# leijue222/Intra-and-Inter-Human-Relation-Network-for-MPEE

Hardware: AMD Instinct MI355X
Metric: images/sec (256x192 crops) I2R-Net HRNet-W48 inference (higher is better)
Workload: dtype f32; 1 GPU; vanilla I2R-Net HRNet-W48-S 256x192, 6 encoder layers, fp32, random weights (BASELINE configs[1]: w48_pure_en6); images_per_gpu=8, persons_per_image=4, crops_per_gpu_step=32, parallelism=single GPU, programs_per_forward=3

## Files before the change

### include/i2r_hip.h

```cpp
#ifndef I2R_HIP_H
#define I2R_HIP_H

#include <stdint.h>

#ifdef __cplusplus
extern "C" {
#endif

#define I2R_ABI_VERSION 17

#define I2R_API __attribute__((visibility("default")))

#define I2R_OK 0
#define I2R_E_ARG (-1)
#define I2R_E_LAUNCH (-2)
#define I2R_E_NODEV (-3)

#define I2R_MAX_TAPS 9

typedef struct i2r_conv_desc {
    const float* in;
    const float* in2;
    const float* w;
    const float* bias;
// ... 39 lines not shown

I2R_API int i2r_pe_res_stem(const float* mask_nchw, const float* w_pre, const float* w7, const float* bias, float* out_nhwc,
                    int32_t n_img, int32_t in_h, int32_t in_w, int32_t cout, int32_t out_cs, int32_t n_src, int32_t n_valid, void* stream);

typedef struct i2r_pe_cat_vec_args {
    const float* in; const float* w; const float* bias; float* out;
    int32_t n_img, in_h, in_w, th, tw, rate, vec, out_cs, c0, c_end, n_src, n_valid;
} i2r_pe_cat_vec_args;
I2R_API int i2r_pe_cat_vec(const i2r_pe_cat_vec_args* a, void* stream);

I2R_API int i2r_maxpool3x3s2(const float* in, float* out, int32_t n_img, int32_t in_h, int32_t in_w, int32_t c,
                     int32_t in_cs, int32_t out_cs, void* stream);

I2R_API int i2r_head(const float* in, const float* w, const float* bias, float* out_nchw, int32_t n_img, int32_t h,
             int32_t w_, int32_t cin, int32_t in_cs, int32_t cout, void* stream);

I2R_API int i2r_conv_kernel_name(const i2r_conv_desc* const* descs, int32_t n, char* buf, int32_t buflen);

I2R_API int i2r_conv_grid(const i2r_conv_desc* const* descs, int32_t n, int32_t with_map, int32_t* grid, int32_t* seq);

I2R_API int i2r_conv_wino_form(const i2r_conv_desc* const* descs, int32_t n, int32_t* form);
I2R_API int i2r_conv_wino_forms(int32_t on);

I2R_API int i2r_flip_merge(const float* y, const float* y_flipped, const int32_t* joint_map, float* out, int32_t n, int32_t joints,
                   int32_t h, int32_t w, void* stream);

I2R_API int i2r_decode(const float* heatmaps, const float* center, const float* scale, float* preds, float* maxvals, int32_t n,
               int32_t joints, int32_t h, int32_t w, int32_t blur_kernel, int32_t transform_back, void* stream);

#define I2R_MAX_TOKEN_TABLES 2
typedef struct i2r_token_table { int32_t* tokens; const int32_t* crop_group; const int32_t* crop_slot; int32_t n_grp, K, fh, fw, down, reserved; } i2r_token_table;
typedef struct i2r_joint_tokens_args {
    const float* heatmaps; float* points; float* maxvals; i2r_token_table table[I2R_MAX_TOKEN_TABLES ];
    int32_t n_crops, joints, hh, hw, in_stride, n_tables;
} i2r_joint_tokens_args;
I2R_API int i2r_joint_tokens(const i2r_joint_tokens_args* a, void* stream);

typedef struct i2r_pose_nms_args {
    const float* preds; const float* maxvals; const float* scale; const float* area; const float* box_score;
    const int32_t* img_off; const float* sigmas;
    float* score; int32_t* rank; int32_t* n_keep;
    double in_vis_thre, oks_thre, oks_vis_thre;
    int32_t n_crops, n_img, joints, max_persons, soft, max_dets, use_oks_vis, reserved;
} i2r_pose_nms_args;
I2R_API int i2r_pose_nms(const i2r_pose_nms_args* a, void* stream);

// ... 289 lines not shown
```

### intra-and-inter-human-relation-network-for-mpee_amd/cabi.py

```python
import ctypes as C
import os

import torch

_HERE = os.path.dirname(os.path.abspath(__file__))
LIB_PATH = os.path.join(_HERE, "libi2r_hip.so")

MAX_TAPS = 9
ABI_VERSION = 17
OP_CONV, OP_STEM, OP_MAXPOOL, OP_HEAD, OP_ENC_KV, OP_ENC_LAYER, OP_FORK, OP_JOIN, OP_CONV_GROUP = 1, 2, 3, 4, 5, 6, 7, 8, 9
MAX_GROUP = 4
OP_LAYERNORM, OP_WINATTN, OP_DWCONV, OP_UPSAMPLE = 10, 11, 12, 13
OP_CONV_CHAIN = 14
OP_PE_RES_STEM = 15
OP_HRT_ATTN = 16
OP_HRT_MLP = 17
OP_XSYNC = 18
OP_FUSE_UP = 19
OP_CONV1X1_PAIR = 20
OP_CONV1X1_LP = 21
OP_MH_ATTN = 22
OP_PE_CAT_VEC = 23
OP_ROWS_GATHER, OP_VIEW_SCRAMBLE = 24, 25
OP_RECORD, OP_WAIT = 26, 27
# ... 213 lines not shown
    _fields_ = [("output", _fp), ("target", _fp), ("target_weight", _fp), ("joints_hm", _fp), ("joints_vis", _fp), ("joints_weight", _fp),
                ("ws", _fp), ("loss", _fp), ("acc", _fp), ("avg_acc", _fp), ("cnt", _fp), ("pred", _fp), ("sse", _fp), ("hits", _fp),
                ("valid", _fp), ("meter", _fp), ("sigma", C.c_double),
                ("n_crops", _i32), ("joints", _i32), ("h", _i32), ("w", _i32), ("use_target_weight", _i32), ("reserved", _i32)]


class ValCombineArgs(C.Structure):
    _fields_ = [("parts", _fp), ("sse", _fp), ("hits", _fp), ("valid", _fp), ("loss", _fp), ("acc", _fp), ("avg_acc", _fp), ("cnt", _fp),
                ("n_crops", _fp), ("meter", _fp), ("n_part", _i32), ("joints", _i32), ("h", _i32), ("w", _i32)]


class ImageRef(C.Structure):
    _fields_ = [("img", C.c_void_p), ("ih", _i32), ("iw", _i32), ("row_bytes", _i32), ("reserved", _i32)]


class CropRef(C.Structure):
    _fields_ = [("inv_m", C.c_double * 6), ("box", _i32 * 4), ("image", _i32), ("reserved", _i32 * 3)]


class Op(C.Structure):
    _fields_ = [("kind", _i32), ("lane", _i32), ("args", C.c_void_p)]


EXPORTS = ("i2r_conv", "i2r_conv_grouped", "i2r_conv_kernel_name", "i2r_conv_grid", "i2r_conv_wino_form", "i2r_conv_wino_forms", "i2r_stem_conv", "i2r_pe_res_stem", "i2r_maxpool3x3s2", "i2r_head", "i2r_layernorm", "i2r_window_attn", "i2r_hrt_attn_block", "i2r_hrt_mlp_block", "i2r_dwconv3x3",
           "i2r_upsample_bilinear_add", "i2r_upsample_bilinear_add_multi", "i2r_fuse_up_add", "i2r_conv1x1_pair", "i2r_conv1x1_lp", "i2r_flip_merge", "i2r_decode", "i2r_joint_tokens", "i2r_pose_nms", "i2r_group_nearest", "i2r_oks_match", "i2r_oks_accumulate", "i2r_joint_targets", "i2r_val_metrics", "i2r_val_combine", "i2r_crop_affine", "i2r_box_mask", "i2r_crop_affine_cv2", "i2r_box_mask_cv2", "i2r_person_inputs_cv2", "i2r_encoder_kv", "i2r_encoder_layer", "i2r_mh_attention", "i2r_attn_weights", "i2r_attn_query_maps", "i2r_attn_person_maps", "i2r_attn_flip_merge", "i2r_token_mirror", "i2r_pe_cat_vec", "i2r_rows_gather", "i2r_rows_gather_multi", "i2r_view_scramble",
           "i2r_run_program", "i2r_run_program_timed", "i2r_abi_version", "i2r_last_error", "i2r_device_check")

_LIB = None


class I2RError(RuntimeError):
    pass


def load_library(path=LIB_PATH):
    if not os.path.exists(path):
        raise I2RError(
            "HIP extension %s is missing -- build it with `python -c 'import __graft_entry__ as g; g.build()'`. "
            "There is no CPU fallback for the product path." % path)
    L = C.CDLL(path)
    L.i2r_conv.argtypes = [C.POINTER(ConvDesc), C.c_void_p]
    L.i2r_conv_grouped.argtypes = [C.POINTER(C.POINTER(ConvDesc)), _i32, _fp, _i32, C.c_void_p]
    L.i2r_conv_kernel_name.argtypes = [C.POINTER(C.POINTER(ConvDesc)), _i32, C.c_char_p, _i32]
    L.i2r_conv_grid.argtypes = [C.POINTER(C.POINTER(ConvDesc)), _i32, _i32, C.POINTER(_i32), C.POINTER(_i32)]
    L.i2r_conv_wino_form.argtypes = [C.POINTER(C.POINTER(ConvDesc)), _i32, C.POINTER(_i32)]
    L.i2r_conv_wino_forms.argtypes = [_i32]
    L.i2r_stem_conv.argtypes = [_fp, _fp, _fp, _fp, _i32, _i32, _i32, _i32, _i32, _i32, _i32, _i32, _i32, C.c_void_p]
    L.i2r_pe_res_stem.argtypes = [_fp, _fp, _fp, _fp, _fp, _i32, _i32, _i32, _i32, _i32, _i32, _i32, C.c_void_p]
    L.i2r_flip_merge.argtypes = [_fp, _fp, _fp, _fp, _i32, _i32, _i32, _i32, C.c_void_p]
    L.i2r_decode.argtypes = [_fp, _fp, _fp, _fp, _fp, _i32, _i32, _i32, _i32, _i32, _i32, C.c_void_p]
    L.i2r_joint_tokens.argtypes = [C.POINTER(JointTokensArgs), C.c_void_p]
    L.i2r_pose_nms.argtypes = [C.POINTER(PoseNmsArgs), C.c_void_p]
    L.i2r_group_nearest.argtypes = [_fp, _fp, _fp, _i32, _i32, _i32, _i32, _fp, C.c_void_p]
    L.i2r_oks_match.argtypes = [C.POINTER(OksMatchArgs), C.c_void_p]
    L.i2r_oks_accumulate.argtypes = [C.POINTER(OksAccumulateArgs), C.c_void_p]
    L.i2r_joint_targets.argtypes = [C.POINTER(JointTargetsArgs), C.c_void_p]
    L.i2r_val_metrics.argtypes = [C.POINTER(ValMetricsArgs), C.c_void_p]
    L.i2r_val_combine.argtypes = [C.POINTER(ValCombineArgs), C.c_void_p]
    L.i2r_crop_affine.argtypes = [_fp, _i32, _i32, _i32, _i32, _fp, _fp, _fp, _fp, _i32, _i32, _i32, C.c_void_p]
    L.i2r_box_mask.argtypes = [_fp, _i32, _i32, _fp, _i32, _i32, _i32, C.c_void_p]
    L.i2r_crop_affine_cv2.argtypes = [_fp, _i32, _i32, _i32, _i32, _fp, _fp, _fp, _fp, _i32, _i32, _i32, C.c_void_p]
    L.i2r_box_mask_cv2.argtypes = [_fp, _i32, _i32, _fp, _i32, _i32, _i32, C.c_void_p]
    L.i2r_person_inputs_cv2.argtypes = [_fp, _i32, _fp, _i32, _i32, C.POINTER(C.c_float), C.POINTER(C.c_float), _fp, _fp, _i32, _i32, C.c_void_p]
    L.i2r_fuse_up_add.argtypes = [_fp, _fp, _i32, _fp, _i32, _fp, _i32, _i32, _i32, _i32, _i32, _i32, C.c_void_p]
    L.i2r_conv1x1_pair.argtypes = [C.POINTER(Conv1x1PairArgs), C.c_void_p]
    L.i2r_conv1x1_lp.argtypes = [C.POINTER(Conv1x1LpArgs), C.c_void_p]
    L.i2r_maxpool3x3s2.argtypes = [_fp, _fp, _i32, _i32, _i32, _i32, _i32, _i32, C.c_void_p]
    L.i2r_head.argtypes = [_fp, _fp, _fp, _fp, _i32, _i32, _i32, _i32, _i32, _i32, C.c_void_p]
    L.i2r_layernorm.argtypes = [_fp, _fp, _fp, _fp, _i32, _i32, _i32, C.c_float, _i32, C.c_void_p]
# ... 49 lines not shown
```

### intra-and-inter-human-relation-network-for-mpee_amd/csrc/i2r_conv.h

```cpp
#pragma once
#include "i2r_common.h"

#ifdef I2R_TUNING
#define I2R_DBG(p) ((p).dbg)
#else
#define I2R_DBG(p) 0
#endif

namespace {

struct ConvK {
    const float* in;
    const float* in2;
    const float* w;
    const float* bias;
    const float* res1;
    const float* res2;
    const float* res_post;
    float* out;
    int n_img, in_h, in_w, in_cs, cin;
    int conv_h, conv_w, out_h, out_w, out_cs, cout, cout_pad;
    int stride, iy0, ix0, ntaps;
    int tap_kh, tap_kw;
    int out_step, out_off_y, out_off_x, rep, relu;
// ... 223 lines not shown
    for (int mt = 0; mt < MT; ++mt) {
        const int m = (wm * MT + mt) * 16 + g * 4 + pj;
        const int ty = div_m(m, p.tile_w, p.m_tw), tx = m - ty * p.tile_w;
        const int oy = oy0 + ty, ox = ox0 + tx;
        const bool pvalid = m < tile_px && oy < p.conv_h && ox < p.conv_w;
        const int by = oy * p.out_step + p.out_off_y, bx = ox * p.out_step + p.out_off_x;
#pragma unroll
        for (int nt = 0; nt < NT; ++nt) {
            const f32x4 v = to_pixel_major(acc[mt][nt]) + bias[nt];
            const int n = n_base + nt * 16 + pq * 4;
            if (!pvalid || noff[nt] == kOOB) continue;
            for (int ry = 0; ry < p.rep; ++ry)
                for (int rx = 0; rx < p.rep; ++rx) {
                    const unsigned o = (unsigned)(((img * p.out_h + by + ry) * p.out_w + bx + rx) * p.out_cs) * esz + noff[nt];
                    f32x4 t = v;
                    if (p.res1) t += buf_ld_act4<DT>(rs_r1, o, h16);
                    if (p.res2) t += buf_ld_act4<DT>(rs_r2, o, h16);
                    buf_st_act4<DT>(rs_out, o, finish(t, n, n + 4 <= p.cout, o), h16);
                }
        }
    }
}



typedef void (*conv_fn)(const ConvGroupK);

}

void* i2r_pick_conv_f32(int nt, int mt, int cap, int pf);
void* i2r_pick_conv_bf16(int nt, int mt, int cap, int pf);
void* i2r_pick_conv_f16(int nt, int mt, int cap, int pf);
void* i2r_pick_conv_wino(int nt, int mt, int fin, int epi);
size_t i2r_conv_wino_lds(int nt, int mt, int plane);
```

### intra-and-inter-human-relation-network-for-mpee_amd/csrc/i2r_conv.hip

```cpp
#include "i2r_conv.h"

namespace {

template <int MT, int NT, int CAP, int PF>
__device__ __forceinline__ void conv_body(const ConvK& p, int bid, f32x4* lds) {
    const int tid = threadIdx.x;
    unsigned long long ts0 = 0, ts1 = 0, ts2 = 0;
    const bool stamp = (I2R_DBG(p) & 8) != 0;
    const int bid_stamp = bid;
    if (stamp) ts0 = __builtin_amdgcn_s_memtime();
    const int lane = tid & 63, wave = tid >> 6;
    const int WN = p.wn;
    const int wm = wave >> p.wn_log, wn = wave & (WN - 1);
    const int li = lane & 15, g = lane >> 4;

    int q = div_m(bid, p.n_cblk, p.m_cblk);
    const int cb = bid - q * p.n_cblk;
    bid = q;
    q = div_m(bid, p.tiles_x, p.m_tx);
    const int tile_x = bid - q * p.tiles_x;
    bid = q;
    const int img = div_m(bid, p.tiles_y, p.m_ty);
    const int tile_y = bid - img * p.tiles_y;
    const int oy0 = tile_y * p.tile_h, ox0 = tile_x * p.tile_w;
// ... 162 lines not shown
    }

    if (stamp) {
        ts2 = __builtin_amdgcn_s_memtime();
        ConvK q = p;
        q.res2 = nullptr;
        conv_epilogue<MT, NT, 0>(q, acc, img, oy0, ox0, wm, n_base, li, g, tile_px);
        asm volatile("s_waitcnt vmcnt(0)" ::: "memory");
        const unsigned long long ts3 = __builtin_amdgcn_s_memtime();
        if (tid == 0) {
            unsigned long long* o = reinterpret_cast<unsigned long long*>(const_cast<float*>(p.res2)) + (size_t)bid_stamp * 4;
            o[0] = ts0; o[1] = ts1; o[2] = ts2; o[3] = ts3;
            if (I2R_DBG(p) & 32) {
                const unsigned hw = __builtin_amdgcn_s_getreg((4 << 0) | (0 << 6) | (31 << 11));
                const unsigned xcc = __builtin_amdgcn_s_getreg((20 << 0) | (0 << 6) | (3 << 11));
                o[1] = ((unsigned long long)xcc << 32) | hw;
            }
        }
        return;
    }
    conv_epilogue<MT, NT, 0>(p, acc, img, oy0, ox0, wm, n_base, li, g, tile_px);
}

template <int MT, int NT, int CAP, int PF>
__global__ __launch_bounds__(256) void conv_igemm_f32(const ConvGroupK grp) {
    extern __shared__ __attribute__((aligned(16))) f32x4 lds[];
    int bid = blockIdx.x, gi = 0, start = 0;
    if (grp.blk_map) {
        const int v = __builtin_amdgcn_readfirstlane(grp.blk_map[bid]);
        gi = v >> 24;
        bid = v & 0xFFFFFF;
    } else {
#pragma unroll
        for (int i = 0; i < kMaxGroups - 1; ++i)
            if (i + 1 < grp.n && bid >= grp.blk_end[i]) { gi = i + 1; start = grp.blk_end[i]; }
    }
    conv_body<MT, NT, CAP, PF>(grp.g[gi], bid - start, lds);
}

template <int NT, int CAP, int PF>
conv_fn pick_mt(int mt) {
    switch (mt) {
        case 1: return conv_igemm_f32<1, NT, CAP, PF>;
        case 2: return conv_igemm_f32<2, NT, CAP, PF>;
        case 3: return conv_igemm_f32<3, NT, CAP, PF>;
        case 4: return conv_igemm_f32<4, NT, CAP, PF>;
    }
    return nullptr;
}

template <int CAP, int PF>
conv_fn pick_nt(int nt, int mt) {
    switch (nt) {
        case 3: return pick_mt<3, CAP, PF>(mt);
        case 4: return pick_mt<4, CAP, PF>(mt);
        case 5: return pick_mt<5, CAP, PF>(mt);
    }
    return nullptr;
}

}

void* i2r_pick_conv_f32(int nt, int mt, int cap, int pf) {
    conv_fn fn = nullptr;
    if (pf == 0) fn = pick_nt<4, 0>(nt, mt);
    if (pf == 1 && cap == 4) fn = pick_nt<4, 1>(nt, mt);
    if (pf == 1 && cap == 12) fn = pick_nt<12, 1>(nt, mt);
    if (pf == 2 && cap == 4) fn = pick_nt<4, 2>(nt, mt);
    return reinterpret_cast<void*>(fn);
}

#include "i2r_conv_plan.h"
```

### intra-and-inter-human-relation-network-for-mpee_amd/csrc/i2r_conv_plan.h

```cpp
#pragma once
#include <stdlib.h>

#include <algorithm>
#include <atomic>

#include "i2r_conv.h"

namespace {

inline int cdiv(int a, int b) { return (a + b - 1) / b; }
inline unsigned magic(int d) { return d == 1 ? 0u : (unsigned)(((1ull << 32) + d - 1) / d); }
inline unsigned recip31(int d) { return (unsigned)(((1ull << 31) + d - 1) / d); }

struct ConvTune { int dbg, plane_pad, pf, cap; };
#ifdef I2R_TUNING
inline const ConvTune& conv_tune() {
    auto env = [](const char* name, int dflt) { const char* v = getenv(name); return v ? atoi(v) : dflt; };
    static const ConvTune t = {env("I2R_CONV_DBG", 0), env("I2R_CONV_PLANE_PAD", 0), env("I2R_CONV_PF", 1), env("I2R_CONV_CAP", 12)};
    return t;
}
#else
constexpr ConvTune conv_tune() { return {0, 0, 1, 12}; }
#endif

struct ConvShape {
    int nt, wn, mt;
    int tile_h, tile_w, tiles_y, tiles_x, n_cblk;
    int tap_kh, tap_kw, ph, pw, plane;
    int npp, cin_g, g_ch;
    int cap, pf, ck;
    unsigned in_bytes, w_bytes, out_bytes;
    size_t lds;
    long long nblk;
};

struct ConvPlan {
    ConvGroupK grp;
    int algo, dtype;
    int nt, mt, cap, pf;
    bool fused_in; int form;
    size_t lds; long long total;
    int seq[kMaxGroups];
    conv_fn fn;
};

void copy_desc(const i2r_conv_desc* d, ConvK& k) {
    k = ConvK{};
    k.in = d->in; k.in2 = d->in2; k.w = d->w; k.bias = d->bias; k.res1 = d->res1; k.res2 = d->res2; k.res_post = d->res_post; k.out = d->out;
    k.n_img = d->n_img; k.in_h = d->in_h; k.in_w = d->in_w; k.in_cs = d->in_cs; k.cin = d->cin;
    k.conv_h = d->conv_h; k.conv_w = d->conv_w; k.out_h = d->out_h; k.out_w = d->out_w; k.out_cs = d->out_cs;
    k.cout = d->cout; k.cout_pad = d->cout_pad; k.stride = d->stride; k.iy0 = d->iy0; k.ix0 = d->ix0; k.ntaps = d->ntaps;
    k.out_step = d->out_step; k.out_off_y = d->out_off_y; k.out_off_x = d->out_off_x; k.rep = d->rep; k.relu = d->relu;
    k.dtype = d->dtype; k.in16 = d->in_f16; k.out16 = d->out_f16;
    k.algo = d->algo; k.w_seq = 1; k.dbg = conv_tune().dbg;
    k.f_t1 = d->t1; k.f_t2 = d->t2; k.f_y = d->y; k.f_sh1 = d->t1_shift; k.f_sh2 = d->t2 ? d->t2_shift : 0;
}

constexpr int kWinoMaxSeq = 8;
constexpr int kWinoRunPasses = 6;
constexpr int kWinoMinWg = 512;
inline int wino_pitch(int fw) { return fw == 8 ? 20 : (fw == 4 ? 10 : 9); }
long long wino_runs(const ConvK& k, int mt) { return (((long long)k.w_nfrag + mt - 1) / mt + k.w_seq - 1) / k.w_seq; }

// ... 211 lines not shown
    k.in_bytes = s.in_bytes; k.out_bytes = s.out_bytes; k.w_bytes = s.w_bytes;
    k.m_cblk = magic(k.n_cblk); k.m_tx = magic(k.tiles_x); k.m_ty = magic(k.tiles_y); k.m_pw = magic(k.pw); k.m_tw = magic(k.tile_w);
    k.wn_log = s.wn == 4 ? 2 : (s.wn == 2 ? 1 : 0);
    k.npass = s.cin_g / (s.ck / s.g_ch);
}

bool any_fused_input(const i2r_conv_desc* const* descs, int32_t n) {
    return std::any_of(descs, descs + n, [](const i2r_conv_desc* d) { return d->t1 != nullptr; });
}

std::atomic<int> g_wino_forms{1};

int wino_form(const i2r_conv_desc* const* descs, int32_t n, const ConvGroupK& grp) {
    if (!g_wino_forms.load(std::memory_order_relaxed)) return 0;
    for (int i = 0; i < n; ++i) {
        const i2r_conv_desc* d = descs[i];
        if (d->relu != 1 || d->res2 || d->res_post || d->cout != d->cout_pad || d->cout_pad > d->out_cs) return 0;
        if ((d->res1 != nullptr) != (descs[0]->res1 != nullptr)) return 0;
        if (I2R_DBG(grp.g[i]) != 0) return 0;
    }
    return descs[0]->res1 ? 2 : 1;
}

int resolve(const i2r_conv_desc* const* descs, int32_t n, bool with_table, ConvPlan& p) {
    I2R_CHECK_ARG(descs && n >= 1 && n <= kMaxGroups, "i2r_conv_grouped: 1..%d descriptors", kMaxGroups);
    for (int i = 0; i < n; ++i) I2R_CHECK_ARG(descs[i] && descs[i]->algo == descs[0]->algo, "i2r_conv_grouped: members mix algorithms");
    ConvShape sh[kMaxGroups];
    ConvGroupK& grp = p.grp;
    auto agrees = [&](int i) -> int {
        I2R_CHECK_ARG(sh[i].nt == sh[0].nt && sh[i].mt == sh[0].mt, "i2r_conv_grouped: descriptor %d has fragment blocking (%d,%d) != (%d,%d)", i,
                      sh[i].mt, sh[i].nt, sh[0].mt, sh[0].nt);
        I2R_CHECK_ARG(descs[i]->dtype == descs[0]->dtype, "i2r_conv_grouped: members mix compute dtypes");
        return I2R_OK;
    };
    const bool settle = n > 1 && descs[0]->algo == 0;
    for (int i = 0; i < n; ++i) {
        int rc = prepare(descs[i], i ? sh[0].mt : 0, sh[i]);
        if (!rc && !settle) rc = agrees(i);
        if (rc) return rc;
    }
    if (settle) {
        int pf = 0, cap = 4;
        bool all_pf = true;
        for (int i = 0; i < n; ++i) {
            all_pf = all_pf && sh[i].pf != 0;
            pf = std::max(pf, sh[i].pf);
// ... 14 lines not shown
    if (p.algo == 1) wino_choose_seq(grp.g, descs, n, p.mt);
    for (int i = 0; i < n; ++i) {
        ConvK& k = grp.g[i];
        long long nblk = sh[i].nblk;
        if (p.algo == 1) {
            const long long runs = wino_runs(k, p.mt);
            nblk = runs * k.n_cblk;
            if (!with_table) {
                k.w_band = (int)((runs + 7) / 8);
                nblk = (long long)k.w_band * 8 * k.n_cblk;
            }
            k.wk.w_seq = k.w_seq; k.wk.w_band = k.w_band;
        }
        p.lds = std::max(p.lds, sh[i].lds);
        p.total += nblk;
        grp.blk_end[i] = (int)p.total;
        p.seq[i] = k.w_seq;
    }
    for (int i = n; i < kMaxGroups; ++i) { grp.g[i] = grp.g[0]; grp.blk_end[i] = (int)p.total; p.seq[i] = 0; }
    grp.n = n; grp.blk_map = nullptr;
    I2R_CHECK_ARG(p.total < (1ll << 31), "i2r_conv_grouped: grid");
    p.fused_in = p.algo == 1 && any_fused_input(descs, n);
    p.form = p.algo == 1 ? wino_form(descs, n, grp) : 0;
    p.fn = reinterpret_cast<conv_fn>(p.algo == 1    ? i2r_pick_conv_wino(p.nt, p.mt, p.fused_in, p.form)
                                     : p.dtype == 0 ? i2r_pick_conv_f32(p.nt, p.mt, p.cap, p.pf)
                                     : p.dtype == 1 ? i2r_pick_conv_bf16(p.nt, p.mt, p.cap, p.pf)
                                                    : i2r_pick_conv_f16(p.nt, p.mt, p.cap, p.pf));
    return I2R_OK;
}

}

extern "C" int i2r_conv_wino_forms(int32_t on) {
    g_wino_forms.store(on ? 1 : 0, std::memory_order_relaxed);
    return I2R_OK;
}

extern "C" int i2r_conv_wino_form(const i2r_conv_desc* const* descs, int32_t n, int32_t* form) {
    ConvPlan p;
    if (int rc = resolve(descs, n, true, p)) return rc;
    I2R_CHECK_ARG(form != nullptr, "i2r_conv_wino_form: form");
    *form = p.form;
    return I2R_OK;
}

extern "C" int i2r_conv_grouped(const i2r_conv_desc* const* descs, int32_t n, const int32_t* block_map, int32_t map_len, void* stream) {
    ConvPlan p;
    if (int rc = resolve(descs, n, block_map != nullptr, p)) return rc;
    p.grp.blk_map = block_map;
    I2R_CHECK_ARG(block_map == nullptr || map_len == (int32_t)p.total, "i2r_conv_grouped: block_map has %d entries, grid has %lld", map_len, p.total);
    I2R_CHECK_ARG(p.fn != nullptr, "i2r_conv: no kernel for nt=%d mt=%d cap=%d pf=%d dtype=%d", p.nt, p.mt, p.cap, p.pf, p.dtype);
    if (p.lds > 64 * 1024)
        (void)hipFuncSetAttribute(reinterpret_cast<const void*>(p.fn), hipFuncAttributeMaxDynamicSharedMemorySize, (int)p.lds);
    i2r_launch(p.fn, dim3((unsigned)p.total), dim3(256), p.lds, (hipStream_t)stream, p.grp);
    I2R_CHECK_LAUNCH("i2r_conv");
    return I2R_OK;
}

extern "C" int i2r_conv(const i2r_conv_desc* d, void* stream) { return i2r_conv_grouped(&d, 1, nullptr, 0, stream); }

extern "C" int i2r_conv_grid(const i2r_conv_desc* const* descs, int32_t n, int32_t with_map, int32_t* grid, int32_t* seq) {
    ConvPlan p;
    if (int rc = resolve(descs, n, with_map != 0, p)) return rc;
    I2R_CHECK_ARG(grid != nullptr, "i2r_conv_grid: grid");
    *grid = (int32_t)p.total;
// ... 17 lines not shown
```

### intra-and-inter-human-relation-network-for-mpee_amd/engine.py

```python
import ctypes as C
import math
import os

import torch

from . import attn_capture, cabi
from .attn_capture import AttnQueries, JointQueries, PersonMaps
from .pack import (PRECISIONS, PackedConv, Packer, _m16, _r16, fold_bn, pack_frag, pack_frag32, pack_k4, pack_k8,
                   winograd_weights)


def wino_fragment(conv_h, conv_w):
    best = None
    for fw in (8, 4, 2):
        n = -(-conv_w // (2 * fw)) * -(-conv_h // (32 // fw))
        if best is None or n < best[0]:
            best = (n, 2 * fw, 32 // fw)
    return best[1], best[2]


LP1X1 = True
LP1X1_MAX_PIX = 65536
_HRT_FUSED_ATTN = (78, 156, 312)
_HRT_FUSED_MLP = (78, 156, 312)
_MLP_VARIANT = {78: 1, 156: 2, 312: 2}
PAIR1X1 = True
FUSE_IN = True
PRUNE_FUSE = True
WINOGRAD = True
WINO_SEQ = True
WINO_FORMS = True
PROFILER_ATTACHED = bool(os.environ.get("ROCP_TOOL_LIBRARIES") or os.environ.get("ROCPROFILER_LIBRARY_CTOR") or os.environ.get("HSA_TOOLS_LIB")
                         or any(t in os.environ.get("LD_PRELOAD", "") for t in ("rocprof", "roctracer", "rocprofiler")))
DEVICE_SYNC = not PROFILER_ATTACHED


class Act:
    __slots__ = ("t", "n", "h", "w", "c", "cs", "dt")
    TORCH_DT = {0: torch.float32, 1: torch.bfloat16, 2: torch.float16}

    def __init__(self, t, n, h, w, c, cs, dt=0):
        self.t, self.n, self.h, self.w, self.c, self.cs, self.dt = t, n, h, w, c, cs, dt

    def view(self):
        return self.t.view(self.TORCH_DT[self.dt])[:self.n * self.h * self.w * self.cs].view(self.n, self.h, self.w, self.cs)

    @property
    def ptr(self):
        return self.t.data_ptr()


class _RawAct:
    __slots__ = ("ptr", "n", "h", "w", "c", "cs", "dt")

# ... 59 lines not shown
        for b in range(n_cu):
            if r < len(bins[b]):
                out.append(bins[b][r])
        r += 1
    return out


def conv_split(cout_pad):
    nfrag = cout_pad // 16
    nt = next(c for c in (3, 4, 5) if nfrag % c == 0)
    nb = nfrag // nt
    wn = 4 if nb % 4 == 0 else 2 if nb % 2 == 0 else 1
    return nt, wn


_wino_forms_pushed = None


def push_wino_forms():
    global _wino_forms_pushed
    if _wino_forms_pushed != bool(WINO_FORMS):
        cabi.check(cabi.lib().i2r_conv_wino_forms(int(bool(WINO_FORMS))), "i2r_conv_wino_forms")
        _wino_forms_pushed = bool(WINO_FORMS)


class Program:
    def __init__(self, device):
        self.device = device
        self.ops = []
        self.keep = []
        self.pool = {}
        self.pending = []
        self.lane_pool = {}
        self.lane_ctx = 0
        self.groupings = []
        self.enc_stacks = []
        self.split_counters = []
        self.captures = []
        self.form = None
        self.store_dt = 0
        self.in_fork = False
        self.nbytes = 0
        self._snap = None
        self._next_slot = -1
        self._c_ops = None
        self._flags_op = None
# ... 657 lines not shown
            self.pool.setdefault(t.numel(), []).append(t)
        for (_, numel), lst in lp.items():
            self.pool.setdefault(numel, []).extend(lst)

    def join(self, mask):
        assert self._snap is None
        self.ops.append((cabi.OP_JOIN, mask, None))
        self.in_fork = False
        self._flush_lane_pools()
        self.lane_ctx = 0

    def finalize(self):
        arr = (cabi.Op * len(self.ops))()
        for i, (kind, lane, st) in enumerate(self.ops):
            arr[i].kind, arr[i].lane = kind, lane
            arr[i].args = C.cast(C.pointer(st), C.c_void_p) if st is not None else None
        self._c_ops = arr
        self._flags_op = next((i for i, (kind, _, _) in enumerate(self.ops) if kind == cabi.OP_LANE_FLAGS), None)
        self.uses_lanes = any(lane != 0 or kind in cabi.SYNC_OPS for kind, lane, _ in self.ops)

    def run(self, side_streams=None, events=None):
        L = cabi.lib()
        push_wino_forms()
        cur = torch.cuda.current_stream(self.device).cuda_stream
        if side_streams is None:
            streams = (C.c_void_p * 4)(cur, cur, cur, cur)
        else:
            streams = (C.c_void_p * 4)(cur, *[s.cuda_stream for s in side_streams])
        evs = None
        if self._flags_op is not None:
            spin = side_streams is not None and DEVICE_SYNC and lanes_independent(self.device, side_streams, cur)
            self._c_ops[self._flags_op].args = self._lane_flags().data_ptr() if spin else None
            self.device_sync = spin
        if self.uses_lanes:
            if events is None:
                events = self._own_events()
            evs = (C.c_void_p * len(events))(*[e.cuda_event for e in events])
        try:
            if Program.timing_log is not None:
                self._run_timed(L, streams, evs)
            else:
                cabi.check(L.i2r_run_program(self._c_ops, len(self.ops), streams, evs), "i2r_run_program")
        except Exception:
            for t in self.split_counters:
                t.zero_()
            raise
# ... 1386 lines not shown
```

Before: 9203 images/sec.

## Add software-pipelined direct f32 conv variants with specialized bias/residual/relu epilogue

Adds a new f32 implicit-GEMM conv body that double-buffers A/B register fragments with sched_barrier fences, so LDS and weight loads overlap MFMA work. It also specializes a single-pass (no LDS double buffer) form. A fused epilogue is specialized for relu with optional residual, and for small MT it prefetches bias and residual loads during the last chunk. A host-side selector picks these forms when the descriptor constraints match, enabled by default, at the cost of more kernel instantiations and higher register pressure.

```diff
diff --git a/include/i2r_hip.h b/include/i2r_hip.h
--- a/include/i2r_hip.h
+++ b/include/i2r_hip.h
@@ -85,6 +85,9 @@
 I2R_API int i2r_conv_wino_form(const i2r_conv_desc* const* descs, int32_t n, int32_t* form);
 I2R_API int i2r_conv_wino_forms(int32_t on);
 
+I2R_API int i2r_conv_direct_form(const i2r_conv_desc* const* descs, int32_t n, int32_t* form, int32_t* epi);
+I2R_API int i2r_conv_direct_forms(int32_t on);
+
 I2R_API int i2r_flip_merge(const float* y, const float* y_flipped, const int32_t* joint_map, float* out, int32_t n, int32_t joints,
                    int32_t h, int32_t w, void* stream);
 
diff --git a/intra-and-inter-human-relation-network-for-mpee_amd/cabi.py b/intra-and-inter-human-relation-network-for-mpee_amd/cabi.py
--- a/intra-and-inter-human-relation-network-for-mpee_amd/cabi.py
+++ b/intra-and-inter-human-relation-network-for-mpee_amd/cabi.py
@@ -259,7 +259,7 @@
     _fields_ = [("kind", _i32), ("lane", _i32), ("args", C.c_void_p)]
 
 
-EXPORTS = ("i2r_conv", "i2r_conv_grouped", "i2r_conv_kernel_name", "i2r_conv_grid", "i2r_conv_wino_form", "i2r_conv_wino_forms", "i2r_stem_conv", "i2r_pe_res_stem", "i2r_maxpool3x3s2", "i2r_head", "i2r_layernorm", "i2r_window_attn", "i2r_hrt_attn_block", "i2r_hrt_mlp_block", "i2r_dwconv3x3",
+EXPORTS = ("i2r_conv", "i2r_conv_grouped", "i2r_conv_kernel_name", "i2r_conv_grid", "i2r_conv_wino_form", "i2r_conv_wino_forms", "i2r_conv_direct_form", "i2r_conv_direct_forms", "i2r_stem_conv", "i2r_pe_res_stem", "i2r_maxpool3x3s2", "i2r_head", "i2r_layernorm", "i2r_window_attn", "i2r_hrt_attn_block", "i2r_hrt_mlp_block", "i2r_dwconv3x3",
            "i2r_upsample_bilinear_add", "i2r_upsample_bilinear_add_multi", "i2r_fuse_up_add", "i2r_conv1x1_pair", "i2r_conv1x1_lp", "i2r_flip_merge", "i2r_decode", "i2r_joint_tokens", "i2r_pose_nms", "i2r_group_nearest", "i2r_oks_match", "i2r_oks_accumulate", "i2r_joint_targets", "i2r_val_metrics", "i2r_val_combine", "i2r_crop_affine", "i2r_box_mask", "i2r_crop_affine_cv2", "i2r_box_mask_cv2", "i2r_person_inputs_cv2", "i2r_encoder_kv", "i2r_encoder_layer", "i2r_mh_attention", "i2r_attn_weights", "i2r_attn_query_maps", "i2r_attn_person_maps", "i2r_attn_flip_merge", "i2r_token_mirror", "i2r_pe_cat_vec", "i2r_rows_gather", "i2r_rows_gather_multi", "i2r_view_scramble",
            "i2r_run_program", "i2r_run_program_timed", "i2r_abi_version", "i2r_last_error", "i2r_device_check")
 
@@ -282,6 +282,8 @@
     L.i2r_conv_grid.argtypes = [C.POINTER(C.POINTER(ConvDesc)), _i32, _i32, C.POINTER(_i32), C.POINTER(_i32)]
     L.i2r_conv_wino_form.argtypes = [C.POINTER(C.POINTER(ConvDesc)), _i32, C.POINTER(_i32)]
     L.i2r_conv_wino_forms.argtypes = [_i32]
+    L.i2r_conv_direct_form.argtypes = [C.POINTER(C.POINTER(ConvDesc)), _i32, C.POINTER(_i32), C.POINTER(_i32)]
+    L.i2r_conv_direct_forms.argtypes = [_i32]
     L.i2r_stem_conv.argtypes = [_fp, _fp, _fp, _fp, _i32, _i32, _i32, _i32, _i32, _i32, _i32, _i32, _i32, C.c_void_p]
     L.i2r_pe_res_stem.argtypes = [_fp, _fp, _fp, _fp, _fp, _i32, _i32, _i32, _i32, _i32, _i32, _i32, C.c_void_p]
     L.i2r_flip_merge.argtypes = [_fp, _fp, _fp, _fp, _i32, _i32, _i32, _i32, C.c_void_p]
diff --git a/intra-and-inter-human-relation-network-for-mpee_amd/csrc/i2r_conv.h b/intra-and-inter-human-relation-network-for-mpee_amd/csrc/i2r_conv.h
--- a/intra-and-inter-human-relation-network-for-mpee_amd/csrc/i2r_conv.h
+++ b/intra-and-inter-human-relation-network-for-mpee_amd/csrc/i2r_conv.h
@@ -269,13 +269,81 @@
     }
 }
 
-
+template <int MT, int NT, int EPI>
+struct ConvEpiPre {
+    __amdgpu_buffer_rsrc_t rs_out, rs_bias, rs_r1;
+    unsigned nb;
+    unsigned off[MT];
+    f32x4 bias[NT];
+    f32x4 r1[EPI == 2 ? MT : 1][NT];
+};
+
+template <int MT, int NT, int EPI>
+__device__ __forceinline__ void conv_epilogue_prep(const ConvK& p, ConvEpiPre<MT, NT, EPI>& pre, int img, int oy0, int ox0, int wm, int n_base,
+                                                   int li, int g, int tile_px) {
+    const int pj = li >> 2, pq = li & 3;
+    float* out = p.out;
+    const float* bias = p.bias;
+    const float* res1 = p.res1;
+    unsigned out_bytes = p.out_bytes, bias_bytes = (unsigned)p.cout_pad * 4u;
+    asm volatile("" : "+s"(out), "+s"(bias), "+s"(res1), "+s"(out_bytes), "+s"(bias_bytes));
+    pre.rs_out = __builtin_amdgcn_make_buffer_rsrc(out, 0, out_bytes, 0x00020000);
+    pre.rs_bias = __builtin_amdgcn_make_buffer_rsrc(const_cast<float*>(bias), 0, bias_bytes, 0x00020000);
+    if constexpr (EPI == 2) pre.rs_r1 = __builtin_amdgcn_make_buffer_rsrc(const_cast<float*>(res1), 0, out_bytes, 0x00020000);
+    pre.nb = (unsigned)(n_base + pq * 4) * 4u;
+    const int conv_h = p.conv_h, conv_w = p.conv_w, out_h = p.out_h, out_w = p.out_w, out_cs = p.out_cs;
+    const int step = p.out_step, off_y = p.out_off_y, off_x = p.out_off_x;
+#pragma unroll
+    for (int mt = 0; mt < MT; ++mt) {
+        const int m = (wm * MT + mt) * 16 + g * 4 + pj;
+        const int ty = div_m(m, p.tile_w, p.m_tw), tx = m - ty * p.tile_w;
+        const int oy = oy0 + ty, ox = ox0 + tx;
+        const bool pv = m < tile_px && oy < conv_h && ox < conv_w;
+        pre.off[mt] = pv ? (unsigned)(((img * out_h + oy * step + off_y) * out_w + ox * step + off_x) * out_cs) * 4u + pre.nb : kOOB;
+        asm volatile("" : "+v"(pre.off[mt]));
+    }
+}
+
+template <int MT, int NT, int EPI>
+__device__ __forceinline__ void conv_epilogue_fetch(ConvEpiPre<MT, NT, EPI>& pre) {
+#pragma unroll
+    for (int nt = 0; nt < NT; ++nt) pre.bias[nt] = buf_ld16(pre.rs_bias, pre.nb + nt * 64u, 0);
+    if constexpr (EPI == 2) {
+#pragma unroll
+        for (int mt = 0; mt < MT; ++mt)
+#pragma unroll
+            for (int nt = 0; nt < NT; ++nt) pre.r1[mt][nt] = buf_ld16(pre.rs_r1, pre.off[mt] + nt * 64u, 0);
+    }
+}
+
+template <int MT, int NT, int EPI>
+__device__ __forceinline__ void conv_epilogue_form(f32x4 (&acc)[MT][NT], const ConvEpiPre<MT, NT, EPI>& pre, int li, int g) {
+    const int j4 = li & 3;
+    const int pj = li >> 2, pq = li & 3;
+    const int perm_src = (g * 16 + pq * 4 + pj) * 4;
+#pragma unroll
+    for (int mt = 0; mt < MT; ++mt)
+#pragma unroll
+        for (int nt = 0; nt < NT; ++nt) {
+            f32x4 v = quad_transpose(acc[mt][nt], j4);
+#pragma unroll
+            for (int e = 0; e < 4; ++e) {
+                const float x = v[e];
+                v[e] = __int_as_float(__builtin_amdgcn_ds_bpermute(perm_src, __float_as_int(x)));
+            }
+            f32x4 r = pre.bias[nt];
+            if constexpr (EPI == 2) r += pre.r1[mt][nt];
+            f32x4 t = v + r;
+            t[0] = fmaxf(t[0], 0.f); t[1] = fmaxf(t[1], 0.f); t[2] = fmaxf(t[2], 0.f); t[3] = fmaxf(t[3], 0.f);
+            buf_st16(pre.rs_out, pre.off[mt] + nt * 64u, 0, t);
+        }
+}
 
 typedef void (*conv_fn)(const ConvGroupK);
 
 }
 
-void* i2r_pick_conv_f32(int nt, int mt, int cap, int pf);
+void* i2r_pick_conv_f32(int nt, int mt, int cap, int pf, int form, int epi);
 void* i2r_pick_conv_bf16(int nt, int mt, int cap, int pf);
 void* i2r_pick_conv_f16(int nt, int mt, int cap, int pf);
 void* i2r_pick_conv_wino(int nt, int mt, int fin, int epi);
diff --git a/intra-and-inter-human-relation-network-for-mpee_amd/csrc/i2r_conv.hip b/intra-and-inter-human-relation-network-for-mpee_amd/csrc/i2r_conv.hip
--- a/intra-and-inter-human-relation-network-for-mpee_amd/csrc/i2r_conv.hip
+++ b/intra-and-inter-human-relation-network-for-mpee_amd/csrc/i2r_conv.hip
@@ -208,7 +208,206 @@
     conv_epilogue<MT, NT, 0>(p, acc, img, oy0, ox0, wm, n_base, li, g, tile_px);
 }
 
-template <int MT, int NT, int CAP, int PF>
+#define CONV_FENCE __builtin_amdgcn_sched_barrier(0);
+template <int MT, int NT, int CAP, int PF, bool SINGLE, int EPI>
+__device__ __forceinline__ void conv_body_forms(const ConvK& p, int bid, f32x4* lds) {
+    static_assert(PF > 0, "the pinned pipeline exists for the double-buffered variants");
+    const int tid = threadIdx.x;
+    const int lane = tid & 63, wave = tid >> 6;
+    const int WN = p.wn;
+    const int wm = wave >> p.wn_log, wn = wave & (WN - 1);
+    const int li = lane & 15, g = lane >> 4;
+
+    int q = div_m(bid, p.n_cblk, p.m_cblk);
+    const int cb = bid - q * p.n_cblk;
+    bid = q;
+    q = div_m(bid, p.tiles_x, p.m_tx);
+    const int tile_x = bid - q * p.tiles_x;
+    bid = q;
+    const int img = div_m(bid, p.tiles_y, p.m_ty);
+    const int tile_y = bid - img * p.tiles_y;
+    const int oy0 = tile_y * p.tile_h, ox0 = tile_x * p.tile_w;
+    const int py0 = oy0 * p.stride + p.iy0, px0 = ox0 * p.stride + p.ix0;
+    const int phw = p.ph * p.pw;
+
+    auto pin = [](int x) __attribute__((always_inline)) { x = __builtin_amdgcn_readfirstlane(x); asm volatile("" : "+s"(x)); return x; };
+    const int plane = pin(p.plane), pw = pin(p.pw), tap_kw = pin(p.tap_kw), cout_slots = pin(p.cout_pad * 16);
+    const int ck = pin(p.ck), npass = pin(p.npass), ntaps = pin(p.ntaps), cin4 = pin(p.cin >> 2);
+    const int ckg = ck >> 2, ncs = ck >> 4, nit = ntaps * ncs;
+
+    constexpr int UQ = CAP / 4, PJ = 4 * PF;
+    const int ul = tid & 3, pp0 = tid >> 2;
+    const __amdgpu_buffer_rsrc_t rs_in = make_rsrc(p.in, p.in_bytes), rs_w = make_rsrc(p.w, p.w_bytes);
+    unsigned goff[PJ];
+#pragma unroll
+    for (int j = 0; j < PJ; ++j) {
+        const int pp = pp0 + j * 64;
+        goff[j] = kOOB;
+        if (pp < phw) {
+            const int py = div_m(pp, p.pw, p.m_pw), px = pp - py * p.pw;
+            const int iy = py0 + py, ix = px0 + px;
+            if (iy >= 0 && iy < p.in_h && ix >= 0 && ix < p.in_w) goff[j] = (unsigned)(((img * p.in_h + iy) * p.in_w + ix) * p.in_cs) * 4u + ul * 16u;
+        }
+    }
+    const int slot0 = ul * plane + pp0;
+
+    const int tile_px = p.tile_h * p.tile_w;
+    int apix[MT];
+#pragma unroll
+    for (int mt = 0; mt < MT; ++mt) {
+        int m = (wm * MT + mt) * 16 + li;
+        if (m >= tile_px) m = 0;
+        const int ty = div_m(m, p.tile_w, p.m_tw), tx = m - ty * p.tile_w;
+        apix[mt] = g * plane + ty * p.stride * pw + tx * p.stride;
+    }
+
+    f32x4 acc[MT][NT];
+#pragma unroll
+    for (int mt = 0; mt < MT; ++mt)
+#pragma unroll
+        for (int nt = 0; nt < NT; ++nt) acc[mt][nt] = (f32x4){0.f, 0.f, 0.f, 0.f};
+
+    const int n_base = (cb * WN + wn) * NT * 16;
+    const unsigned wlane = (unsigned)(n_base + li + g * p.cout_pad) * 16u;
+
+    const int w_cs = 4 * cout_slots, w_dtap = (cin4 - ncs * 4) * cout_slots;
+    const int a_cs = 4 * plane, a_dtap = 1 - ncs * 4 * plane, a_drow = pw - tap_kw;
+
+    unsigned oob[UQ];
+#pragma unroll
+    for (int uq = 0; uq < UQ; ++uq) oob[uq] = uq * 4 < ckg ? 0u : kOOB;
+    f32x4 v[UQ][PJ];
+    auto stage_load = [&](int c0) __attribute__((always_inline)) {
+#pragma unroll
+        for (int uq = 0; uq < UQ; ++uq)
+#pragma unroll
+            for (int j = 0; j < PJ; ++j) v[uq][j] = buf_ld16(rs_in, uq == 0 ? goff[j] : ((goff[j] + uq * 64u) | oob[uq]), c0 * 4);
+    };
+    auto stage_store = [&](f32x4* buf) __attribute__((always_inline)) {
+#pragma unroll
+        for (int uq = 0; uq < UQ; ++uq)
+#pragma unroll
+            for (int j = 0; j < PJ; ++j) asm volatile("" : "+v"(v[uq][j]));
+#pragma unroll
+        for (int uq = 0; uq < UQ; ++uq)
+            if (uq * 4 < ckg) {
+                f32x4* q4 = buf + uq * 4 * plane + slot0;
+#pragma unroll
+                for (int j = 0; j < PJ; ++j)
+                    if (pp0 + j * 64 < phw) q4[j * 64] = v[uq][j];
+            }
+    };
+
+    f32x4 a0[MT], a1[MT], b0[NT], b1[NT];
+    int wp = 0, cs_b = 0;
+    int ao = 0, cs_a = 0, tx_a = 0;
+    auto fetch_b = [&](f32x4(&b)[NT]) __attribute__((always_inline)) {
+#pragma unroll
+        for (int nt = 0; nt < NT; ++nt) b[nt] = buf_ld16(rs_w, wlane + nt * 256u, wp);
+        const bool wc = cs_b + 1 == ncs;
+        cs_b = wc ? 0 : cs_b + 1;
+        wp += w_cs + (wc ? w_dtap : 0);
+    };
+    auto fetch_a = [&](const f32x4* buf, f32x4(&a)[MT]) __attribute__((always_inline)) {
+        const f32x4* qa = buf + ao;
+#pragma unroll
+        for (int mt = 0; mt < MT; ++mt) a[mt] = qa[apix[mt]];
+        const bool wc = cs_a + 1 == ncs;
+        const bool wx = wc && tx_a + 1 == tap_kw;
+        cs_a = wc ? 0 : cs_a + 1;
+        tx_a = wx ? 0 : tx_a + (wc ? 1 : 0);
+        ao += a_cs + (wc ? a_dtap : 0) + (wx ? a_drow : 0);
+    };
+    auto first_b = [&](int c0) __attribute__((always_inline)) {
+        wp = (c0 >> 2) * cout_slots;
+        cs_b = 0;
+        fetch_b(b0);
+    };
+    auto fma_step = [&](const f32x4(&a)[MT], const f32x4(&b)[NT]) __attribute__((always_inline)) {
+#pragma unroll
+        for (int s = 0; s < 4; ++s)
+#pragma unroll
+            for (int mt = 0; mt < MT; ++mt)
+#pragma unroll
+                for (int nt = 0; nt < NT; ++nt) acc[mt][nt] = mfma16(a[mt][s], b[nt][s], acc[mt][nt]);
+    };
+
+    auto run_chunk = [&](const f32x4* buf, auto&& tail) __attribute__((always_inline)) {
+        ao = 0; cs_a = 0; tx_a = 0;
+        fetch_a(buf, a0);
+        CONV_FENCE
+        int it = 0;
+        for (; it + 4 <= nit; it += 2) {
+            fetch_b(b1); fetch_a(buf, a1);
+            CONV_FENCE
+            fma_step(a0, b0);
+            CONV_FENCE
+            fetch_b(b0); fetch_a(buf, a0);
+            CONV_FENCE
+            fma_step(a1, b1);
+            CONV_FENCE
+        }
+        const int rem = nit - it;
+        if (rem == 3) {
+            fetch_b(b1); fetch_a(buf, a1);
+            CONV_FENCE
+            fma_step(a0, b0);
+            CONV_FENCE
+            fetch_b(b0); fetch_a(buf, a0);
+            tail();
+            CONV_FENCE
+            fma_step(a1, b1);
+            CONV_FENCE
+            fma_step(a0, b0);
+        } else if (rem == 2) {
+            fetch_b(b1); fetch_a(buf, a1);
+            tail();
+            CONV_FENCE
+            fma_step(a0, b0);
+            CONV_FENCE
+            fma_step(a1, b1);
+        } else {
+            tail();
+            CONV_FENCE
+            fma_step(a0, b0);
+        }
+        CONV_FENCE
+    };
+
+    constexpr bool EARLY = EPI != 0 && MT <= 2;
+    ConvEpiPre<MT, NT, EPI == 0 ? 1 : EPI> pre;
+    if constexpr (EPI != 0) conv_epilogue_prep<MT, NT, EPI>(p, pre, img, oy0, ox0, wm, n_base, li, g, tile_px);
+    auto last_tail = [&]() __attribute__((always_inline)) {
+        if constexpr (EARLY) conv_epilogue_fetch<MT, NT, EPI>(pre);
+    };
+
+    stage_load(0);
+    first_b(0);
+    stage_store(lds);
+    __syncthreads();
+    if constexpr (SINGLE) {
+        run_chunk(lds, last_tail);
+    } else {
+        const int bufsz = ckg * plane;
+        int pass = 0;
+        for (; pass + 1 < npass; ++pass) {
+            run_chunk(lds + (pass & 1) * bufsz, [&]() __attribute__((always_inline)) { stage_load((pass + 1) * ck); });
+            first_b((pass + 1) * ck);
+            stage_store(lds + ((pass + 1) & 1) * bufsz);
+            __syncthreads();
+        }
+        run_chunk(lds + (pass & 1) * bufsz, last_tail);
+    }
+
+    if constexpr (EPI == 0) {
+        conv_epilogue<MT, NT, 0>(p, acc, img, oy0, ox0, wm, n_base, li, g, tile_px);
+    } else {
+        if constexpr (!EARLY) conv_epilogue_fetch<MT, NT, EPI>(pre);
+        conv_epilogue_form<MT, NT, EPI>(acc, pre, li, g);
+    }
+}
+
+template <int MT, int NT, int CAP, int PF, int FORM = 0, int EPI = 0>
 __global__ __launch_bounds__(256) void conv_igemm_f32(const ConvGroupK grp) {
     extern __shared__ __attribute__((aligned(16))) f32x4 lds[];
     int bid = blockIdx.x, gi = 0, start = 0;
@@ -221,39 +420,63 @@
         for (int i = 0; i < kMaxGroups - 1; ++i)
             if (i + 1 < grp.n && bid >= grp.blk_end[i]) { gi = i + 1; start = grp.blk_end[i]; }
     }
-    conv_body<MT, NT, CAP, PF>(grp.g[gi], bid - start, lds);
-}
-
-template <int NT, int CAP, int PF>
+    if constexpr (FORM == 0)
+        conv_body<MT, NT, CAP, PF>(grp.g[gi], bid - start, lds);
+    else
+        conv_body_forms<MT, NT, CAP, PF, FORM == 1, EPI>(grp.g[gi], bid - start, lds);
+}
+
+#ifdef I2R_CONV_KERNELS_ONLY
+}
+#else
+template <int NT, int CAP, int PF, int FORM, int EPI>
 conv_fn pick_mt(int mt) {
     switch (mt) {
-        case 1: return conv_igemm_f32<1, NT, CAP, PF>;
-        case 2: return conv_igemm_f32<2, NT, CAP, PF>;
-        case 3: return conv_igemm_f32<3, NT, CAP, PF>;
-        case 4: return conv_igemm_f32<4, NT, CAP, PF>;
+        case 1: return conv_igemm_f32<1, NT, CAP, PF, FORM, EPI>;
+        case 2: return conv_igemm_f32<2, NT, CAP, PF, FORM, EPI>;
+        case 3: return conv_igemm_f32<3, NT, CAP, PF, FORM, EPI>;
+        case 4:
+            if constexpr (FORM == 0) return conv_igemm_f32<4, NT, CAP, PF, 0, 0>;
     }
     return nullptr;
 }
 
-template <int CAP, int PF>
+template <int CAP, int PF, int FORM, int EPI>
 conv_fn pick_nt(int nt, int mt) {
     switch (nt) {
-        case 3: return pick_mt<3, CAP, PF>(mt);
-        case 4: return pick_mt<4, CAP, PF>(mt);
-        case 5: return pick_mt<5, CAP, PF>(mt);
+        case 3: return pick_mt<3, CAP, PF, FORM, EPI>(mt);
+        case 4: return pick_mt<4, CAP, PF, FORM, EPI>(mt);
+        case 5: return pick_mt<5, CAP, PF, FORM, EPI>(mt);
     }
     return nullptr;
 }
 
-}
-
-void* i2r_pick_conv_f32(int nt, int mt, int cap, int pf) {
+template <int FORM, int EPI>
+conv_fn pick_variant(int nt, int mt, int cap, int pf) {
+    if constexpr (FORM == 0) {
+        if (pf == 0) return pick_nt<4, 0, 0, 0>(nt, mt);
+    }
+    if (pf == 1 && cap == 4) return pick_nt<4, 1, FORM, EPI>(nt, mt);
+    if (pf == 1 && cap == 12) return pick_nt<12, 1, FORM, EPI>(nt, mt);
+    if (pf == 2 && cap == 4) return pick_nt<4, 2, FORM, EPI>(nt, mt);
+    return nullptr;
+}
+
+}
+
+void* i2r_pick_conv_f32(int nt, int mt, int cap, int pf, int form, int epi) {
     conv_fn fn = nullptr;
-    if (pf == 0) fn = pick_nt<4, 0>(nt, mt);
-    if (pf == 1 && cap == 4) fn = pick_nt<4, 1>(nt, mt);
-    if (pf == 1 && cap == 12) fn = pick_nt<12, 1>(nt, mt);
-    if (pf == 2 && cap == 4) fn = pick_nt<4, 2>(nt, mt);
+    switch (form * 3 + epi) {
+        case 0: fn = pick_variant<0, 0>(nt, mt, cap, pf); break;
+        case 3: fn = pick_variant<1, 0>(nt, mt, cap, pf); break;
+        case 4: fn = pick_variant<1, 1>(nt, mt, cap, pf); break;
+        case 5: fn = pick_variant<1, 2>(nt, mt, cap, pf); break;
+        case 6: fn = pick_variant<2, 0>(nt, mt, cap, pf); break;
+        case 7: fn = pick_variant<2, 1>(nt, mt, cap, pf); break;
+        case 8: fn = pick_variant<2, 2>(nt, mt, cap, pf); break;
+    }
     return reinterpret_cast<void*>(fn);
 }
 
 #include "i2r_conv_plan.h"
+#endif
diff --git a/intra-and-inter-human-relation-network-for-mpee_amd/csrc/i2r_conv_plan.h b/intra-and-inter-human-relation-network-for-mpee_amd/csrc/i2r_conv_plan.h
--- a/intra-and-inter-human-relation-network-for-mpee_amd/csrc/i2r_conv_plan.h
+++ b/intra-and-inter-human-relation-network-for-mpee_amd/csrc/i2r_conv_plan.h
@@ -39,6 +39,7 @@
     int algo, dtype;
     int nt, mt, cap, pf;
     bool fused_in; int form;
+    int dform, depi;
     size_t lds; long long total;
     int seq[kMaxGroups];
     conv_fn fn;
@@ -296,6 +297,25 @@
     return descs[0]->res1 ? 2 : 1;
 }
 
+std::atomic<int> g_direct_forms{1};
+constexpr int kDirectFormMaxMT = 3;
+
+void direct_form(const i2r_conv_desc* const* descs, int32_t n, const ConvGroupK& grp, int pf, int mt, int& form, int& epi) {
+    form = epi = 0;
+    if (pf == 0 || mt > kDirectFormMaxMT || descs[0]->algo != 0 || descs[0]->dtype != 0 || !g_direct_forms.load(std::memory_order_relaxed)) return;
+    for (int i = 0; i < n; ++i)
+        if (I2R_DBG(grp.g[i]) != 0 || descs[i]->in2) return;
+    form = 1;
+    epi = descs[0]->res1 ? 2 : 1;
+    for (int i = 0; i < n; ++i) {
+        const i2r_conv_desc* d = descs[i];
+        if (grp.g[i].npass != 1) form = 2;
+        if (d->relu != 1 || d->res2 || d->res_post || d->rep != 1 || d->cout != d->cout_pad || d->cout_pad > d->out_cs ||
+            (d->res1 != nullptr) != (descs[0]->res1 != nullptr))
+            epi = 0;
+    }
+}
+
 int resolve(const i2r_conv_desc* const* descs, int32_t n, bool with_table, ConvPlan& p) {
     I2R_CHECK_ARG(descs && n >= 1 && n <= kMaxGroups, "i2r_conv_grouped: 1..%d descriptors", kMaxGroups);
     for (int i = 0; i < n; ++i) I2R_CHECK_ARG(descs[i] && descs[i]->algo == descs[0]->algo, "i2r_conv_grouped: members mix algorithms");
@@ -356,8 +376,9 @@
     I2R_CHECK_ARG(p.total < (1ll << 31), "i2r_conv_grouped: grid");
     p.fused_in = p.algo == 1 && any_fused_input(descs, n);
     p.form = p.algo == 1 ? wino_form(descs, n, grp) : 0;
+    direct_form(descs, n, grp, p.pf, p.mt, p.dform, p.depi);
     p.fn = reinterpret_cast<conv_fn>(p.algo == 1    ? i2r_pick_conv_wino(p.nt, p.mt, p.fused_in, p.form)
-                                     : p.dtype == 0 ? i2r_pick_conv_f32(p.nt, p.mt, p.cap, p.pf)
+                                     : p.dtype == 0 ? i2r_pick_conv_f32(p.nt, p.mt, p.cap, p.pf, p.dform, p.depi)
                                      : p.dtype == 1 ? i2r_pick_conv_bf16(p.nt, p.mt, p.cap, p.pf)
                                                     : i2r_pick_conv_f16(p.nt, p.mt, p.cap, p.pf));
     return I2R_OK;
@@ -375,6 +396,20 @@
     if (int rc = resolve(descs, n, true, p)) return rc;
     I2R_CHECK_ARG(form != nullptr, "i2r_conv_wino_form: form");
     *form = p.form;
+    return I2R_OK;
+}
+
+extern "C" int i2r_conv_direct_forms(int32_t on) {
+    g_direct_forms.store(on ? 1 : 0, std::memory_order_relaxed);
+    return I2R_OK;
+}
+
+extern "C" int i2r_conv_direct_form(const i2r_conv_desc* const* descs, int32_t n, int32_t* form, int32_t* epi) {
+    ConvPlan p;
+    if (int rc = resolve(descs, n, true, p)) return rc;
+    I2R_CHECK_ARG(form != nullptr, "i2r_conv_direct_form: form");
+    *form = p.dform;
+    if (epi) *epi = p.depi;
     return I2R_OK;
 }
 
diff --git a/intra-and-inter-human-relation-network-for-mpee_amd/engine.py b/intra-and-inter-human-relation-network-for-mpee_amd/engine.py
--- a/intra-and-inter-human-relation-network-for-mpee_amd/engine.py
+++ b/intra-and-inter-human-relation-network-for-mpee_amd/engine.py
@@ -30,6 +30,7 @@
 WINOGRAD = True
 WINO_SEQ = True
 WINO_FORMS = True
+CONV_FORMS = True
 PROFILER_ATTACHED = bool(os.environ.get("ROCP_TOOL_LIBRARIES") or os.environ.get("ROCPROFILER_LIBRARY_CTOR") or os.environ.get("HSA_TOOLS_LIB")
                          or any(t in os.environ.get("LD_PRELOAD", "") for t in ("rocprof", "roctracer", "rocprofiler")))
 DEVICE_SYNC = not PROFILER_ATTACHED
@@ -135,6 +136,16 @@
     if _wino_forms_pushed != bool(WINO_FORMS):
         cabi.check(cabi.lib().i2r_conv_wino_forms(int(bool(WINO_FORMS))), "i2r_conv_wino_forms")
         _wino_forms_pushed = bool(WINO_FORMS)
+
+
+_conv_forms_pushed = None
+
+
+def push_conv_forms():
+    global _conv_forms_pushed
+    if _conv_forms_pushed != bool(CONV_FORMS):
+        cabi.check(cabi.lib().i2r_conv_direct_forms(int(bool(CONV_FORMS))), "i2r_conv_direct_forms")
+        _conv_forms_pushed = bool(CONV_FORMS)
 
 
 class Program:
@@ -838,6 +849,7 @@
     def run(self, side_streams=None, events=None):
         L = cabi.lib()
         push_wino_forms()
+        push_conv_forms()
         cur = torch.cuda.current_stream(self.device).cuda_stream
         if side_streams is None:
             streams = (C.c_void_p * 4)(cur, cur, cur, cur)
```

Result: faster. 9305 images/sec, median of 6 (+1.1%).
